# akavkl/Automated-Recycling-Sorter-with-Vision-Transformers

Measured on NVIDIA B200. Metric: vit_b16_224_inference_images_per_sec, higher is better.
Workload: dtype bf16

## Files before the change

automated-recycling-sorter-with-vision-transformers_b200/csrc/common.cu:

```cuda
#include "common.h"

#include <cstdarg>
#include <cstring>
#include <atomic>
#include <mutex>
#include <vector>

namespace vitk {

static thread_local char g_err[1024] = "";
static std::atomic<long long> g_launches{0};

int set_error(int code, const char* fmt, ...) {
  va_list ap;
  va_start(ap, fmt);
  vsnprintf(g_err, sizeof(g_err), fmt, ap);
  va_end(ap);
  return code;
}
const char* last_error() { return g_err; }

void count_launch() { g_launches.fetch_add(1, std::memory_order_relaxed); }
long long launch_count() { return g_launches.load(std::memory_order_relaxed); }

// ... 86 lines not shown
  cudaGetDevice(&dev);
  if (!g_dev_init[dev]) init_dev(dev);
  const int n = g_sm_count[dev] - g_sm_reserve;
  return n < 2 ? 2 : n;
}
int device_cc() {
  int dev = 0;
  cudaGetDevice(&dev);
  if (!g_dev_init[dev]) init_dev(dev);
  return g_cc[dev];
}

typedef CUresult (*EncodeTiledFn)(CUtensorMap*, CUtensorMapDataType, cuuint32_t, void*,
                                  const cuuint64_t*, const cuuint64_t*, const cuuint32_t*,
                                  const cuuint32_t*, CUtensorMapInterleave, CUtensorMapSwizzle,
                                  CUtensorMapL2promotion, CUtensorMapFloatOOBfill);
static EncodeTiledFn g_encode = nullptr;
static std::once_flag g_encode_once;

static EncodeTiledFn get_encode() {
  std::call_once(g_encode_once, [] {
    void* fn = nullptr;
    cudaDriverEntryPointQueryResult qres;
    if (cudaGetDriverEntryPoint("cuTensorMapEncodeTiled", &fn, cudaEnableDefault, &qres) ==
            cudaSuccess &&
        qres == cudaDriverEntryPointSuccess)
      g_encode = reinterpret_cast<EncodeTiledFn>(fn);
  });
  return g_encode;
}

int make_tmap_2d(CUtensorMap* out, const void* base, int elem_bytes, uint64_t inner,
                 uint64_t outer, uint64_t pitch_bytes, uint32_t box_inner, uint32_t box_outer,
                 bool swizzle128) {
  EncodeTiledFn enc = get_encode();
  if (!enc) return set_error(VITK_ERR_CUDA, "cuTensorMapEncodeTiled entry point not available");
  if ((reinterpret_cast<uintptr_t>(base) & 15) != 0 || (pitch_bytes & 15) != 0)
    return set_error(VITK_ERR_INVALID,
                     "TMA operand must be 16-byte aligned (base %p, pitch %llu bytes)", base,
                     (unsigned long long)pitch_bytes);
  if (box_inner * (uint32_t)elem_bytes > 128 && swizzle128)
    return set_error(VITK_ERR_INVALID, "128B-swizzled TMA box inner extent exceeds 128 bytes");
  if (box_outer > 256 || box_inner > 256)
    return set_error(VITK_ERR_INVALID, "TMA box extent exceeds 256");
  CUtensorMapDataType dt;
  switch (elem_bytes) {
    case 2: dt = CU_TENSOR_MAP_DATA_TYPE_BFLOAT16; break;
    case 4: dt = CU_TENSOR_MAP_DATA_TYPE_FLOAT32; break;
    default: return set_error(VITK_ERR_INVALID, "unsupported TMA element size %d", elem_bytes);
  }
  cuuint64_t dims[2] = {inner, outer};
  cuuint64_t strides[1] = {pitch_bytes};
  cuuint32_t box[2] = {box_inner, box_outer};
  cuuint32_t estr[2] = {1, 1};
  CUresult r = enc(out, dt, 2, const_cast<void*>(base), dims, strides, box, estr,
                   CU_TENSOR_MAP_INTERLEAVE_NONE,
                   swizzle128 ? CU_TENSOR_MAP_SWIZZLE_128B : CU_TENSOR_MAP_SWIZZLE_NONE,
                   CU_TENSOR_MAP_L2_PROMOTION_L2_256B, CU_TENSOR_MAP_FLOAT_OOB_FILL_NONE);
  if (r != CUDA_SUCCESS)
    return set_error(VITK_ERR_CUDA,
                     "cuTensorMapEncodeTiled failed (%d): base %p dims {%llu,%llu} pitch %llu box "
                     "{%u,%u}",
                     (int)r, base, (unsigned long long)inner, (unsigned long long)outer,
                     (unsigned long long)pitch_bytes, box_inner, box_outer);
  return VITK_OK;
}

int make_tmap_3d(CUtensorMap* out, const void* base, int elem_bytes, uint64_t inner, uint64_t rows,
                 uint64_t batch, uint64_t row_pitch_bytes, uint64_t batch_pitch_bytes,
                 uint32_t box_inner, uint32_t box_rows) {
  EncodeTiledFn enc = get_encode();
  if (!enc) return set_error(VITK_ERR_CUDA, "cuTensorMapEncodeTiled entry point not available");
  if ((reinterpret_cast<uintptr_t>(base) & 15) != 0 || (row_pitch_bytes & 15) != 0 ||
      (batch_pitch_bytes & 15) != 0)
    return set_error(VITK_ERR_INVALID, "TMA operand must be 16-byte aligned");
  if (box_inner * (uint32_t)elem_bytes != 128 || box_rows > 256 || box_rows == 0)
    return set_error(VITK_ERR_INVALID, "bad 3-D TMA box {%u,%u}", box_inner, box_rows);
  CUtensorMapDataType dt;
  switch (elem_bytes) {
    case 2: dt = CU_TENSOR_MAP_DATA_TYPE_BFLOAT16; break;
    case 4: dt = CU_TENSOR_MAP_DATA_TYPE_FLOAT32; break;
    default: return set_error(VITK_ERR_INVALID, "unsupported TMA element size %d", elem_bytes);
  }
  cuuint64_t dims[3] = {inner, rows, batch};
  cuuint64_t strides[2] = {row_pitch_bytes, batch_pitch_bytes};
  cuuint32_t box[3] = {box_inner, box_rows, 1};
  cuuint32_t estr[3] = {1, 1, 1};
  CUresult r = enc(out, dt, 3, const_cast<void*>(base), dims, strides, box, estr,
                   CU_TENSOR_MAP_INTERLEAVE_NONE, CU_TENSOR_MAP_SWIZZLE_128B,
                   CU_TENSOR_MAP_L2_PROMOTION_L2_256B, CU_TENSOR_MAP_FLOAT_OOB_FILL_NONE);
  if (r != CUDA_SUCCESS)
// ... 6 lines not shown
```

automated-recycling-sorter-with-vision-transformers_b200/csrc/common.h:

```cpp
#pragma once
#include <cstddef>
#include <cstdint>
#include <cstdio>
#include <cuda.h>
#include <cuda_runtime.h>

#include "../../include/vitk.h"

namespace vitk {


int set_error(int code, const char* fmt, ...);
const char* last_error();

#define VITK_CHECK_CUDA(expr)                                                              \
  do {                                                                                     \
    cudaError_t _e = (expr);                                                               \
    if (_e != cudaSuccess)                                                                 \
      return ::vitk::set_error(VITK_ERR_CUDA, "%s failed: %s (%s:%d)", #expr,      \
                               cudaGetErrorString(_e), __FILE__, __LINE__);                \
  } while (0)

#define VITK_CHECK_LAUNCH(name)                                                            \
  do {                                                                                     \
// ... 26 lines not shown
  explicit Carver(void* b) : base(static_cast<char*>(b)) {}
  void* take(size_t n) {
    void* p = base ? base + off : nullptr;
    off += align_up(n, 1024);
    return p;
  }
};

enum ProfKind : int { PROF_GEMM = 0, PROF_ATTN = 1, PROF_LN = 2, PROF_PATCH = 3, PROF_OTHER = 4,
                      PROF_OPT = 5, PROF_NKINDS = 6 };
bool profile_enabled();
void profile_enable(bool on);
int profile_collect(double* ms, double* work, long long* launches, int nkinds);

struct ProfileScope {
  ProfileScope(int kind, double work, cudaStream_t stream);
  ~ProfileScope();
  int idx_;
  cudaStream_t stream_;
};

struct SweepAlternation {
  SweepAlternation();
  ~SweepAlternation();
};
int sweep_next();

int sm_count();
void reserve_sms(int n);
int device_cc();

int make_tmap_2d(CUtensorMap* out, const void* base, int elem_bytes, uint64_t inner,
                 uint64_t outer, uint64_t pitch_bytes, uint32_t box_inner, uint32_t box_outer,
                 bool swizzle128 = true);

int make_tmap_3d(CUtensorMap* out, const void* base, int elem_bytes, uint64_t inner, uint64_t rows,
                 uint64_t batch, uint64_t row_pitch_bytes, uint64_t batch_pitch_bytes,
                 uint32_t box_inner, uint32_t box_rows);

}
```

automated-recycling-sorter-with-vision-transformers_b200/csrc/gemm_sm100.cu:

```cuda
#include "gemm_sm100.cuh"

#include <mutex>

#include "common.h"
#include "ptx.cuh"
#include "rowops.cuh"
#include "train_ops.cuh"

namespace vitk {
using namespace ptx;

#ifdef VITK_GEMM_TRACE
__device__ long long g_gemm_trace[160][8];
#define GT_BEGIN(v) const long long v = clock64()
#define GT_ADD(acc, v) acc += clock64() - v
#else
#define GT_BEGIN(v) do { } while (0)
#define GT_ADD(acc, v) do { } while (0)
#endif

namespace {

constexpr int kBlockM = 128;
constexpr int kBlockK = 64;
constexpr int kUmmaK = 16;
constexpr int kNumEpiWarps = 8;
constexpr int kFirstEpiWarp = 4;
constexpr int kNumThreads = (kFirstEpiWarp + kNumEpiWarps) * 32;
constexpr int kAccStages = 2;

template <int BLOCK_N, int CTAS, int SLABS = 2>
struct Cfg {
  static constexpr int kStagingPerWarp = SLABS * 4096;
  static constexpr int kStagingBytes = kNumEpiWarps * kStagingPerWarp;
  static constexpr int kABytes = kBlockM * kBlockK * 2;
  static constexpr int kBRows = BLOCK_N / CTAS;
  static constexpr int kBBytes = kBRows * kBlockK * 2;
  static constexpr int kStageBytes = kABytes + kBBytes;
  static constexpr int kBarBytes = 1024;
  static constexpr int kBudget = 232448 - 1024 - kBarBytes - kStagingBytes;
  static constexpr int kStages = kBudget / kStageBytes > 8 ? 8 : kBudget / kStageBytes;
  static constexpr int kTmemCols = kAccStages * BLOCK_N;
  static constexpr int kSmemBytes =
      kStages * kStageBytes + kStagingBytes + kBarBytes + 1024;
  static_assert(kStages >= 3, "pipeline too shallow");
  static_assert(kSmemBytes <= 232448, "exceeds 227 KB of shared memory");
  static constexpr int kNumBars = 2 * kStages + 2 * kAccStages + 1 + 2 * kNumEpiWarps;
  static_assert(8 * kNumBars <= kBarBytes, "barrier block too small");
};

__device__ __forceinline__ float gelu_erf(float x) {
  return 0.5f * x * (1.f + erff(x * 0.70710678118654752440f));
}
__device__ __forceinline__ float gelu_fast(float x) {
  const float x2 = fminf(x * x, 100.f);
  const float p = fmaf(x2, fmaf(x2, 9.2473074e-4f, -0.10595751f), -2.3019681f);
  float e, r;
  asm("ex2.approx.ftz.f32 %0, %1;" : "=f"(e) : "f"(x * p));
  asm("rcp.approx.ftz.f32 %0, %1;" : "=f"(r) : "f"(1.f + e));
  return x * r;
}
__device__ __forceinline__ float gelu_fast_tanh(float x) {
  const float x2 = fminf(x * x, 64.f);
  const float p = fmaf(x2, fmaf(x2, -3.5651449e-4f, 0.037011533f), 0.79753114f);
  float t;
  asm("tanh.approx.f32 %0, %1;" : "=f"(t) : "f"(x * p));
  return x * fmaf(0.5f, t, 0.5f);
}
__device__ __forceinline__ float gelu_grad_fast(float x) {
  const float x2 = fminf(x * x, 100.f);
  const float p = fmaf(x2, fmaf(x2, 9.2473074e-4f, -0.10595751f), -2.3019681f);
  float e, phi;
  asm("ex2.approx.ftz.f32 %0, %1;" : "=f"(e) : "f"(x * p));
  asm("rcp.approx.ftz.f32 %0, %1;" : "=f"(phi) : "f"(1.f + e));
  const float gp = fmaf(x2, fmaf(x2, -3.20487363e-3f, 0.22033243f), 1.5956033f);
  return fmaf(x * phi, (1.f - phi) * gp, phi);
}
__device__ __forceinline__ void gelu_fast_tanh_pair(float& a, float& b) {
// ... 188 lines not shown
        o.x = x[4 * j + 0] + r.x;
        o.y = x[4 * j + 1] + r.y;
        o.z = x[4 * j + 2] + r.z;
        o.w = x[4 * j + 3] + r.w;
        reinterpret_cast<float4*>(out)[j] = o;
      }
    } else {
      _Pragma("unroll") for (int j = 0; j < 32; ++j)
        if (n0 + j < N) out[j] = x[j] + res[j];
    }
  } else if constexpr (EPI == EPI_F32) {
    float* out = reinterpret_cast<float*>(e.out) + static_cast<size_t>(m) * e.ldo + n0;
    const float beta = e.beta;
    if (full) {
#pragma unroll
      for (int j = 0; j < 8; ++j) {
        float4 o = make_float4(x[4 * j + 0], x[4 * j + 1], x[4 * j + 2], x[4 * j + 3]);
        if (beta != 0.f) {
          const float4 p = reinterpret_cast<const float4*>(out)[j];
          o.x = fmaf(beta, p.x, o.x);
          o.y = fmaf(beta, p.y, o.y);
          o.z = fmaf(beta, p.z, o.z);
          o.w = fmaf(beta, p.w, o.w);
        }
        reinterpret_cast<float4*>(out)[j] = o;
      }
    } else {
      _Pragma("unroll") for (int j = 0; j < 32; ++j)
        if (n0 + j < N) out[j] = (beta != 0.f) ? fmaf(beta, out[j], x[j]) : x[j];
    }
  }
}

template <int EPI>
__device__ __forceinline__ void acc_plus_bias(const uint32_t (&v)[32], int n0, int N,
                                              const GemmEpilogue& e, float (&x)[32]) {
  float acc_scale = 1.f;
  if constexpr (EPI == EPI_F32) acc_scale = e.alpha;
  if (n0 + 32 <= N) {
    if (e.bias != nullptr) {
      const float4* b4 = reinterpret_cast<const float4*>(e.bias + n0);
#pragma unroll
      for (int j = 0; j < 8; ++j) {
        const float4 b = __ldg(b4 + j);
#ifdef VITK_SCALAR_BIAS
        if constexpr (true) {
#else
        if constexpr (EPI == EPI_F32) {
#endif
          x[4 * j + 0] = fmaf(acc_scale, __uint_as_float(v[4 * j + 0]), b.x);
          x[4 * j + 1] = fmaf(acc_scale, __uint_as_float(v[4 * j + 1]), b.y);
          x[4 * j + 2] = fmaf(acc_scale, __uint_as_float(v[4 * j + 2]), b.z);
          x[4 * j + 3] = fmaf(acc_scale, __uint_as_float(v[4 * j + 3]), b.w);
        } else {
          unpack2(fadd2(pack2(v[4 * j + 0], v[4 * j + 1]), pack2f(b.x, b.y)), x[4 * j + 0],
                  x[4 * j + 1]);
          unpack2(fadd2(pack2(v[4 * j + 2], v[4 * j + 3]), pack2f(b.z, b.w)), x[4 * j + 2],
                  x[4 * j + 3]);
        }
      }
    } else {
#pragma unroll
      for (int j = 0; j < 32; ++j) x[j] = acc_scale * __uint_as_float(v[j]);
    }
  } else {
#pragma unroll
    for (int j = 0; j < 32; ++j) {
      const float b = (e.bias != nullptr && n0 + j < N) ? __ldg(e.bias + n0 + j) : 0.f;
      x[j] = fmaf(acc_scale, __uint_as_float(v[j]), b);
    }
  }
}

__device__ __forceinline__ void acc_scale_bias(const uint32_t (&v)[32], int n0, int N,
                                               const GemmEpilogue& e, float rstd, float (&x)[32]) {
  if (n0 + 32 <= N) {
    const float4* b4 = reinterpret_cast<const float4*>(e.bias + n0);
    const uint64_t r2 = pack2f(rstd, rstd);
#pragma unroll
    for (int j = 0; j < 8; ++j) {
      const float4 b = __ldg(b4 + j);
      unpack2(ffma2(r2, pack2(v[4 * j + 0], v[4 * j + 1]), pack2f(b.x, b.y)), x[4 * j + 0],
              x[4 * j + 1]);
      unpack2(ffma2(r2, pack2(v[4 * j + 2], v[4 * j + 3]), pack2f(b.z, b.w)), x[4 * j + 2],
              x[4 * j + 3]);
    }
  } else {
#pragma unroll
    for (int j = 0; j < 32; ++j) {
      const float b = (n0 + j < N) ? __ldg(e.bias + n0 + j) : 0.f;
      x[j] = fmaf(rstd, __uint_as_float(v[j]), b);
    }
  }
}

__device__ __forceinline__ void resid_chunk_staged(const uint32_t (&v)[32], int row0, int n0, int M,
                                                   int N, const GemmEpilogue& e, uint32_t slab,
                                                   int lane) {
  float x[32];
  acc_plus_bias<EPI_RESID_F32>(v, n0, N, e, x);
  if (e.drop.thresh != 0u)
    drop_apply_run<32>(x, static_cast<uint32_t>(row0 + lane) * static_cast<uint32_t>(N) +
                              static_cast<uint32_t>(n0), e.drop);
  const uint32_t row = slab + static_cast<uint32_t>(lane) * 128u;
#pragma unroll
  for (int j = 0; j < 8; ++j)
    st_shared_v4(row + (static_cast<uint32_t>(j ^ (lane & 7)) << 4), __float_as_uint(x[4 * j]),
                 __float_as_uint(x[4 * j + 1]), __float_as_uint(x[4 * j + 2]),
                 __float_as_uint(x[4 * j + 3]));
  __syncwarp();
  const int piece = lane & 7;
  const bool col_ok = n0 + 4 * piece < N;
  const bool vec_ok = aligned16(e.out) && aligned16(e.resid);
#pragma unroll
  for (int it = 0; it < 8; ++it) {
    const int r = it * 4 + (lane >> 3);
    const int m = row0 + r;
    if (m < M && col_ok) {
      int out_row = m, res_row = m;
      if (e.rows_per_group > 0) {
        const int g = m / e.rows_per_group;
        const int rr = m - g * e.rows_per_group;
// ... 16 lines not shown
        o[0] = a0 + rs[0];
        o[1] = a1 + rs[1];
        o[2] = a2 + rs[2];
        o[3] = a3 + rs[3];
      }
    }
  }
  __syncwarp();
}

__device__ __forceinline__ void stage_and_store(const uint32_t (&pk)[32], uint32_t stg, int& buf,
                                                int lane, const CUtensorMap* tmap, int c0, int c1,
                                                bool reduce) {
  if (lane == 0) tma_store_wait_read<1>();
  __syncwarp();
  const uint32_t slab = stg + static_cast<uint32_t>(buf) * 4096u;
  const uint32_t row = slab + static_cast<uint32_t>(lane) * 128u;
#pragma unroll
  for (int j = 0; j < 8; ++j)
    st_shared_v4(row + (static_cast<uint32_t>(j ^ (lane & 7)) << 4), pk[4 * j], pk[4 * j + 1],
                 pk[4 * j + 2], pk[4 * j + 3]);
  fence_proxy_async_smem();
  __syncwarp();
  if (lane == 0) {
    if (reduce)
      tma_reduce_add_2d(tmap, slab, c0, c1);
    else
      tma_store_2d(tmap, slab, c0, c1);
    tma_store_commit();
  }
  buf ^= 1;
}

template <int BLOCK_N, int EPI, int CTAS, bool TMA_EPI, bool MN>
__global__ void __launch_bounds__(kNumThreads, 1)
gemm_tn_kernel(const __grid_constant__ CUtensorMap tmap_a,
               const __grid_constant__ CUtensorMap tmap_b,
               const __grid_constant__ CUtensorMap tmap_c,
               const __grid_constant__ CUtensorMap tmap_c2, int M, int N, int K,
               int kb_per_split, int num_splits, int descending,
               const __grid_constant__ GemmEpilogue e) {
  constexpr bool kAuxTma = TMA_EPI && (EPI == EPI_DGELU_BF16);
  constexpr bool kStats = TMA_EPI && (EPI == EPI_RESID_STATS_F32);
  static_assert(EPI != EPI_RESID_STATS_F32 || TMA_EPI, "the statistics epilogue is TMA-only");
  using C = Cfg<BLOCK_N, CTAS, kAuxTma ? 3 : 2>;
  constexpr int kStagingBytes = C::kStagingBytes;
  constexpr int kStagingPerWarp = C::kStagingPerWarp;
  constexpr int kTileM = kBlockM * CTAS;
  extern __shared__ uint8_t smem_raw[];
  const uint32_t raw_addr = smem_u32(smem_raw);
  const uint32_t base = (raw_addr + 1023u) & ~1023u;
  uint8_t* smem = smem_raw + (base - raw_addr);

  const uint32_t staging_base = base + C::kStages * C::kStageBytes;
  const uint32_t bar_base = staging_base + kStagingBytes;
  auto full_bar = [&](int s) { return bar_base + 8u * s; };
  auto empty_bar = [&](int s) { return bar_base + 8u * (C::kStages + s); };
  auto tfull_bar = [&](int a) { return bar_base + 8u * (2 * C::kStages + a); };
  auto tempty_bar = [&](int a) { return bar_base + 8u * (2 * C::kStages + kAccStages + a); };
  volatile uint32_t* tmem_slot = reinterpret_cast<volatile uint32_t*>(
      smem + C::kStages * C::kStageBytes + kStagingBytes + 8 * (2 * C::kStages + 2 * kAccStages));
  auto aux_bar = [&](int w) { return bar_base + 8u * (2 * C::kStages + 2 * kAccStages + 1 + w); };
  [[maybe_unused]] auto aux2_bar = [&](int w) {
    return bar_base + 8u * (2 * C::kStages + 2 * kAccStages + 1 + kNumEpiWarps + w);
  };

  const int warp = threadIdx.x >> 5;
  const int lane = threadIdx.x & 31;
  const uint32_t cta_rank = (CTAS == 2) ? cluster_ctarank() : 0u;
  const bool is_leader = (cta_rank == 0);
  const int cluster_id = blockIdx.x / CTAS;
  const int num_clusters = gridDim.x / CTAS;

  const int num_m_tiles = (M + kTileM - 1) / kTileM;
  const int num_n_tiles = (N + BLOCK_N - 1) / BLOCK_N;
  const int num_out_tiles = num_m_tiles * num_n_tiles;
  const int num_tiles = num_out_tiles * num_splits;
  const int num_kb_total = (K + kBlockK - 1) / kBlockK;
// ... 78 lines not shown
                tma_load_2d(sa + j * 8192, &tmap_a, fbar, m0 + 64 * j, kb * kBlockK);
            }
#pragma unroll
            for (int j = 0; j < C::kBRows / 64; ++j) {
              if constexpr (CTAS == 2)
                tma_load_2d_2sm(sb + j * 8192, &tmap_b, fbar, n0 + 64 * j, kb * kBlockK);
              else
                tma_load_2d(sb + j * 8192, &tmap_b, fbar, n0 + 64 * j, kb * kBlockK);
            }
          }
          if (++stage == C::kStages) {
            stage = 0;
            phase ^= 1u;
          }
        }
      }
      if constexpr (CTAS == 2) {
        for (int s = 0; s < C::kStages; ++s) {
          mbar_wait(empty_bar(stage), phase ^ 1u);
          if (++stage == C::kStages) {
            stage = 0;
            phase ^= 1u;
          }
        }
      }
    }
  } else if (warp == 1) {
    if (is_leader) {
      constexpr uint32_t idesc = make_idesc_bf16(kTileM, BLOCK_N, MN ? 1 : 0, MN ? 1 : 0);
      int stage = 0;
      uint32_t phase = 0;
      int acc = 0;
      uint32_t acc_phase = 0;
      [[maybe_unused]] long long gt_full = 0, gt_empty = 0;
      GT_BEGIN(gt_start);
      for (int work = cluster_id; work < num_tiles; work += num_clusters) {
        GT_BEGIN(gt_e);
        mbar_wait(tempty_bar(acc), acc_phase ^ 1u);
        GT_ADD(gt_empty, gt_e);
        tc_fence_after();
        const uint32_t d_tmem = tmem_base + static_cast<uint32_t>(acc * BLOCK_N);
        const int kb0 = kb_begin(work);
        for (int kb = kb0; kb < kb_end(work); ++kb) {
          GT_BEGIN(gt_f);
          mbar_wait(full_bar(stage), phase);
          GT_ADD(gt_full, gt_f);
          tc_fence_after();
          const uint32_t sa = base + stage * C::kStageBytes;
          const uint32_t sb = sa + C::kABytes;
          const uint64_t a_desc = make_desc_sw128(sa, MN ? 8192 : 16, 1024);
          const uint64_t b_desc = make_desc_sw128(sb, MN ? 8192 : 16, 1024);
          constexpr uint32_t kstep = MN ? 128u : 2u;
          if (elect_one_sync()) {
#pragma unroll
            for (int k = 0; k < kBlockK / kUmmaK; ++k) {
              const uint32_t accum = (kb > kb0 || k > 0) ? 1u : 0u;
              if constexpr (CTAS == 2)
                mma_bf16_ss_2sm(d_tmem, a_desc + kstep * k, b_desc + kstep * k, idesc, accum);
              else
                mma_bf16_ss(d_tmem, a_desc + kstep * k, b_desc + kstep * k, idesc, accum);
            }
            if constexpr (CTAS == 2) mma_commit_2sm_mc(empty_bar(stage), 3);
            else mma_commit(empty_bar(stage));
          }
          __syncwarp();
          if (++stage == C::kStages) {
            stage = 0;
            phase ^= 1u;
          }
        }
        if (elect_one_sync()) {
          if constexpr (CTAS == 2) mma_commit_2sm_mc(tfull_bar(acc), 3);
          else mma_commit(tfull_bar(acc));
        }
        __syncwarp();
        if (++acc == kAccStages) {
          acc = 0;
          acc_phase ^= 1u;
        }
      }
#ifdef VITK_GEMM_TRACE
      if (lane == 0 && cluster_id < 160) {
        g_gemm_trace[cluster_id][0] = clock64() - gt_start;
        g_gemm_trace[cluster_id][1] = gt_full;
        g_gemm_trace[cluster_id][2] = gt_empty;
        g_gemm_trace[cluster_id][3] = (num_tiles - cluster_id + num_clusters - 1) / num_clusters;
      }
#endif
    }
  } else if (warp >= kFirstEpiWarp) {
    const int q = warp & 3;
    const int half = (warp - kFirstEpiWarp) >> 2;
    constexpr int kColsPerWarp = BLOCK_N / 2;
    const int slab_row = static_cast<int>(cta_rank) * kBlockM + q * 32;
    const uint32_t stg = staging_base + static_cast<uint32_t>(warp - kFirstEpiWarp) * kStagingPerWarp;
    int buf = 0;
    int acc = 0;
    uint32_t acc_phase = 0;
    [[maybe_unused]] uint32_t aux_phase = 0;
    [[maybe_unused]] const uint32_t aux_slab = stg + 2u * 4096u;
    [[maybe_unused]] const uint32_t my_aux_bar = aux_bar(warp - kFirstEpiWarp);
    [[maybe_unused]] const uint32_t my_aux2_bar = aux2_bar(warp - kFirstEpiWarp);
    [[maybe_unused]] uint32_t x_phase = 0;
    [[maybe_unused]] long long gt_epi_wait = 0, gt_epi_ld = 0, gt_epi_math = 0, gt_epi_store = 0;
    [[maybe_unused]] float2 ln_next[8];
    [[maybe_unused]] float ln_rstd_next = 1.f;
    [[maybe_unused]] bool ln_have_next = false;
    [[maybe_unused]] auto ln_load_stats = [&](int m, float2 (&t)[8]) {
#pragma unroll
      for (int p2 = 0; p2 < 8; ++p2) {
        t[p2] = make_float2(0.f, 0.f);
        if (p2 < e.ln_nparts && m < M)
          asm volatile("ld.global.nc.v2.f32 {%0, %1}, [%2];"
                       : "=f"(t[p2].x), "=f"(t[p2].y)
                       : "l"(e.ln_part + static_cast<size_t>(p2) * M + m));
      }
    };
    [[maybe_unused]] auto ln_finish = [&](float s1, float s2) {
      const float inv_d = 1.f / static_cast<float>(e.ln_dim);
      const float mean = s1 * inv_d;
      const float var = fmaxf(fmaf(-mean, mean, s2 * inv_d), 0.f);
      return rsqrtf(var + e.ln_eps);
    };
    for (int work = cluster_id; work < num_tiles; work += num_clusters) {
      const int tile = tile_of(work);
      const int m_blk = tile / num_n_tiles;
      const int n_blk = tile - m_blk * num_n_tiles;
      if constexpr (kAuxTma) {
        const int r0 = m_blk * kTileM + slab_row;
        const int c0 = n_blk * BLOCK_N + half * kColsPerWarp;
        if (lane == 0 && r0 < M && c0 < N) {
          mbar_arrive_expect_tx(my_aux_bar, 4096);
          tma_load_2d(aux_slab, &tmap_c2, my_aux_bar, c0, r0);
        }
      }
      const int row0 = m_blk * kTileM + slab_row;
      if constexpr (kStats) {
        if (lane == 0 && row0 < M) {
          tma_store_wait_read<0>();
#pragma unroll
          for (int c = 0; c < 2; ++c) {
            const int c0 = n_blk * BLOCK_N + half * kColsPerWarp + 32 * c;
            if (c0 < N) {
              const uint32_t xb = c == 0 ? my_aux_bar : my_aux2_bar;
              mbar_arrive_expect_tx(xb, 4096);
              tma_load_2d(stg + static_cast<uint32_t>(c) * 4096u, &tmap_c, xb, c0, row0);
            }
          }
        }
      }
      [[maybe_unused]] float ln_rstd = 1.f;
      if constexpr (TMA_EPI && (EPI == EPI_BF16 || is_gelu_epi<EPI>())) {
        if (e.ln_part != nullptr) {
          if (ln_have_next) {
            ln_rstd = ln_rstd_next;
          } else {
            float s1 = 0.f, s2 = 0.f;
            ln_load_stats(row0 + lane, ln_next);
#pragma unroll
            for (int p2 = 0; p2 < 8; ++p2) {
              s1 += ln_next[p2].x;
              s2 += ln_next[p2].y;
            }
            ln_rstd = ln_finish(s1, s2);
          }
          const int work_nx = work + num_clusters;
          ln_have_next = work_nx < num_tiles;
          if (ln_have_next)
            ln_load_stats((tile_of(work_nx) / num_n_tiles) * kTileM + slab_row + lane, ln_next);
        }
      }
      GT_BEGIN(gt_w);
      mbar_wait(tfull_bar(acc), acc_phase);
      GT_ADD(gt_epi_wait, gt_w);
      tc_fence_after();
      const uint32_t t_row = tmem_base + (static_cast<uint32_t>(q * 32) << 16) +
                             static_cast<uint32_t>(acc * BLOCK_N + half * kColsPerWarp);
      const int n_base = n_blk * BLOCK_N + half * kColsPerWarp;
      auto release_acc = [&]() {
        tc_fence_before();
        __syncwarp();
        if (lane == 0) {
          if (CTAS == 2 && !is_leader)
            mbar_arrive_cluster(mapa_shared(tempty_bar(acc), 0));
          else
            mbar_arrive(tempty_bar(acc));
        }
      };
      if constexpr (kStats) {
        const bool o2_wide =
            ((reinterpret_cast<uintptr_t>(e.out2) | static_cast<uintptr_t>(e.ldo * 2)) & 31u) == 0;
        float sum1 = 0.f, sum2 = 0.f;
        uint32_t v[2][32];
        tmem_ld_32x32b_x32(t_row, v[0]);
#pragma unroll
        for (int c = 0; c < kColsPerWarp / 32; ++c) {
          tmem_ld_wait();
          if (c + 1 < kColsPerWarp / 32) tmem_ld_32x32b_x32(t_row + (c + 1) * 32, v[(c + 1) & 1]);
          else release_acc();
          const int n0 = n_base + c * 32;
          if (row0 < M && n0 < N) {
            float x[32];
            acc_plus_bias<EPI>(v[c & 1], n0, N, e, x);
            const uint32_t slab = stg + static_cast<uint32_t>(c & 1) * 4096u;
            const uint32_t row = slab + static_cast<uint32_t>(lane) * 128u;
            mbar_wait((c & 1) ? my_aux2_bar : my_aux_bar, (x_phase >> (c & 1)) & 1u);
            x_phase ^= 1u << (c & 1);
#pragma unroll
            for (int j = 0; j < 8; ++j) {
              float r0, r1, r2, r3;
              asm volatile("ld.shared.v4.f32 {%0,%1,%2,%3}, [%4];"
// ... 55 lines not shown
              const uint32_t xb = (c & 1) ? my_aux2_bar : my_aux_bar;
              mbar_arrive_expect_tx(xb, 4096);
              tma_load_2d(slab, &tmap_c, xb, n0 + 64, row0);
            }
          }
        }
        if (row0 + lane < M && n_base < N)
          e.ln_part_out[static_cast<size_t>(n_base / kColsPerWarp) * M + (row0 + lane)] =
              make_float2(sum1, sum2);
      } else if constexpr (TMA_EPI) {
        constexpr bool kOutF32 = (EPI == EPI_RESID_F32 || EPI == EPI_F32);
        if constexpr (kOutF32) {
          const bool reduce = (EPI == EPI_RESID_F32) || (e.beta != 0.f);
          uint32_t v[2][32];
          tmem_ld_32x32b_x32(t_row, v[0]);
#pragma unroll
          for (int c = 0; c < kColsPerWarp / 32; ++c) {
            tmem_ld_wait();
            if (c + 1 < kColsPerWarp / 32) tmem_ld_32x32b_x32(t_row + (c + 1) * 32, v[(c + 1) & 1]);
            else release_acc();
            const int n0 = n_base + c * 32;
            if (row0 < M && n0 < N) {
              float x[32];
              acc_plus_bias<EPI>(v[c & 1], n0, N, e, x);
              if constexpr (EPI == EPI_RESID_F32) {
                if (e.drop.thresh != 0u)
                  drop_apply_run<32>(x, static_cast<uint32_t>(row0 + lane) * static_cast<uint32_t>(N) +
                                            static_cast<uint32_t>(n0), e.drop);
              }
              uint32_t pk[32];
#pragma unroll
              for (int j = 0; j < 32; ++j) pk[j] = __float_as_uint(x[j]);
              stage_and_store(pk, stg, buf, lane, &tmap_c, n0, row0, reduce);
            }
          }
        } else {
#pragma unroll 1
          for (int g = 0; g < kColsPerWarp / 64; ++g) {
            uint32_t v0[32], v1[32];
            GT_BEGIN(gt_l);
            tmem_ld_32x32b_x32(t_row + g * 64, v0);
            tmem_ld_32x32b_x32(t_row + g * 64 + 32, v1);
            tmem_ld_wait();
            if (g + 1 == kColsPerWarp / 64) release_acc();
            GT_ADD(gt_epi_ld, gt_l);
            GT_BEGIN(gt_m);
            const int n0 = n_base + g * 64;
            if (row0 < M && n0 < N) {
              float x0[32], x1[32];
              if (e.ln_part != nullptr) {
                acc_scale_bias(v0, n0, N, e, ln_rstd, x0);
                acc_scale_bias(v1, n0 + 32, N, e, ln_rstd, x1);
              } else {
                acc_plus_bias<EPI>(v0, n0, N, e, x0);
                acc_plus_bias<EPI>(v1, n0 + 32, N, e, x1);
              }
              uint32_t pk[32];
              [[maybe_unused]] const uint32_t drop_idx0 =
                  static_cast<uint32_t>(row0 + lane) * static_cast<uint32_t>(N) +
                  static_cast<uint32_t>(n0);
              if constexpr (EPI == EPI_DGELU_BF16) {
                if (e.drop.thresh != 0u) {
                  drop_apply_run<32>(x0, drop_idx0, e.drop);
                  drop_apply_run<32>(x1, drop_idx0 + 32u, e.drop);
                }
              }
              if constexpr (kAuxTma) {
                mbar_wait(my_aux_bar, aux_phase);
                aux_phase ^= 1u;
                uint32_t a[32];
                const uint32_t arow = aux_slab + static_cast<uint32_t>(lane) * 128u;
#pragma unroll
                for (int j = 0; j < 8; ++j)
                  asm volatile("ld.shared.v4.b32 {%0,%1,%2,%3}, [%4];"
                               : "=r"(a[4 * j]), "=r"(a[4 * j + 1]), "=r"(a[4 * j + 2]),
                                 "=r"(a[4 * j + 3])
                               : "r"(arow + (static_cast<uint32_t>(j ^ (lane & 7)) << 4))
                               : "memory");
                __syncwarp();
                const int n_next = n0 + 64;
                if (lane == 0 && g + 1 < kColsPerWarp / 64 && n_next < N) {
                  mbar_arrive_expect_tx(my_aux_bar, 4096);
                  tma_load_2d(aux_slab, &tmap_c2, my_aux_bar, n_next, row0);
                }
#pragma unroll
                for (int j = 0; j < 16; ++j) {
                  dgelu_tanh_pair(x0[2 * j], x0[2 * j + 1], bf16lo_to_f32(a[j]), bf16hi_to_f32(a[j]));
                  dgelu_tanh_pair(x1[2 * j], x1[2 * j + 1], bf16lo_to_f32(a[16 + j]),
                                  bf16hi_to_f32(a[16 + j]));
                }
              }
              if constexpr (is_gelu_epi<EPI>()) {
                if (e.out2 != nullptr) {
#pragma unroll
                  for (int j = 0; j < 16; ++j) {
                    pk[j] = pack_bf16x2(x0[2 * j], x0[2 * j + 1]);
                    pk[16 + j] = pack_bf16x2(x1[2 * j], x1[2 * j + 1]);
                  }
                  stage_and_store(pk, stg, buf, lane, &tmap_c2, n0, row0, false);
                }
                if constexpr (EPI == EPI_RELU_BF16) {
#pragma unroll
                  for (int j = 0; j < 32; ++j) {
                    x0[j] = fmaxf(x0[j], 0.f);
                    x1[j] = fmaxf(x1[j], 0.f);
                  }
                } else if constexpr (EPI == EPI_GELU_TANH_BF16) {
#pragma unroll
                  for (int j = 0; j < 16; ++j) {
                    gelu_fast_tanh_pair(x0[2 * j], x0[2 * j + 1]);
                    gelu_fast_tanh_pair(x1[2 * j], x1[2 * j + 1]);
                  }
                } else {
#pragma unroll
                  for (int j = 0; j < 16; ++j) {
                    gelu_fast_pair(x0[2 * j], x0[2 * j + 1]);
                    gelu_fast_pair(x1[2 * j], x1[2 * j + 1]);
                  }
                }
                if (e.drop.thresh != 0u) {
                  drop_apply_run<32>(x0, drop_idx0, e.drop);
                  drop_apply_run<32>(x1, drop_idx0 + 32u, e.drop);
                }
              }
#pragma unroll
              for (int j = 0; j < 16; ++j) {
                pk[j] = pack_bf16x2(x0[2 * j], x0[2 * j + 1]);
                pk[16 + j] = pack_bf16x2(x1[2 * j], x1[2 * j + 1]);
              }
              GT_ADD(gt_epi_math, gt_m);
              GT_BEGIN(gt_s);
              stage_and_store(pk, stg, buf, lane, &tmap_c, n0, row0, false);
              GT_ADD(gt_epi_store, gt_s);
            }
          }
        }
      } else {
        const int m = row0 + lane;
        uint32_t v[2][32];
        tmem_ld_32x32b_x32(t_row, v[0]);
#pragma unroll
        for (int c = 0; c < kColsPerWarp / 32; ++c) {
          tmem_ld_wait();
          if (c + 1 < kColsPerWarp / 32) tmem_ld_32x32b_x32(t_row + (c + 1) * 32, v[(c + 1) & 1]);
          else release_acc();
          const int n0 = n_base + c * 32;
          if constexpr (EPI == EPI_RESID_F32) {
            if (row0 < M && n0 < N) resid_chunk_staged(v[c & 1], row0, n0, M, N, e, stg, lane);
          } else {
            if (m < M && n0 < N) epilogue_chunk<EPI>(v[c & 1], m, n0, N, e);
          }
// ... 12 lines not shown
            s2 += ln_next[p2].y;
          }
          ln_rstd_next = ln_finish(s1, s2);
        }
      }
    }
#ifdef VITK_GEMM_TRACE
    if (lane == 0 && warp == kFirstEpiWarp && is_leader && cluster_id < 160) {
      g_gemm_trace[cluster_id][4] = gt_epi_wait;
      g_gemm_trace[cluster_id][5] = gt_epi_ld;
      g_gemm_trace[cluster_id][6] = gt_epi_math;
      g_gemm_trace[cluster_id][7] = gt_epi_store;
    }
#endif
    if constexpr (TMA_EPI) {
      if (lane == 0) tma_store_wait<0>();
    }
  }

  tc_fence_before();
  if constexpr (CTAS == 2) cluster_sync_all(); else __syncthreads();
  if (warp == 2) {
    tc_fence_after();
    if constexpr (CTAS == 2) tmem_dealloc_2sm(tmem_base, C::kTmemCols);
    else tmem_dealloc(tmem_base, C::kTmemCols);
  }
}

int g_force_ctas = 0;
int g_force_direct_epi = 0;

template <int BLOCK_N, int EPI, int CTAS, bool TMA_EPI, bool MN>
int launch(const GemmProblem& p, cudaStream_t stream) {
  using C = Cfg<BLOCK_N, CTAS, (TMA_EPI && EPI == EPI_DGELU_BF16) ? 3 : 2>;
  auto kernel = gemm_tn_kernel<BLOCK_N, EPI, CTAS, TMA_EPI, MN>;
  static std::once_flag once;
  static cudaError_t attr_err = cudaSuccess;
  std::call_once(once, [&] {
    attr_err = cudaFuncSetAttribute(kernel, cudaFuncAttributeMaxDynamicSharedMemorySize,
                                    C::kSmemBytes);
  });
  if (attr_err != cudaSuccess)
    return set_error(VITK_ERR_CUDA, "cudaFuncSetAttribute(gemm smem %d) failed: %s", C::kSmemBytes,
                     cudaGetErrorString(attr_err));
  CUtensorMap ta, tb, tc, tc2;
  if constexpr (MN) {
    VITK_TRY(make_tmap_2d(&ta, p.A, 2, (uint64_t)p.M, (uint64_t)p.K, (uint64_t)p.lda * 2, 64, 64));
    VITK_TRY(make_tmap_2d(&tb, p.B, 2, (uint64_t)p.N, (uint64_t)p.K, (uint64_t)p.ldb * 2, 64, 64));
  } else {
    VITK_TRY(make_tmap_2d(&ta, p.A, 2, (uint64_t)p.K, (uint64_t)p.M, (uint64_t)p.lda * 2, kBlockK,
                          kBlockM));
    VITK_TRY(make_tmap_2d(&tb, p.B, 2, (uint64_t)p.K, (uint64_t)p.N, (uint64_t)p.ldb * 2, kBlockK,
                          C::kBRows));
  }
  if constexpr (TMA_EPI) {
    constexpr bool kOutF32 =
        (EPI == EPI_RESID_F32 || EPI == EPI_F32 || EPI == EPI_RESID_STATS_F32);
    constexpr int eb = kOutF32 ? 4 : 2;
    VITK_TRY(make_tmap_2d(&tc, p.e.out, eb, (uint64_t)p.N, (uint64_t)p.M, (uint64_t)p.e.ldo * eb,
                          128 / eb, 32));
    tc2 = tc;
    if (is_gelu_epi<EPI>() && p.e.out2 != nullptr)
      VITK_TRY(make_tmap_2d(&tc2, p.e.out2, eb, (uint64_t)p.N, (uint64_t)p.M,
                            (uint64_t)p.e.ldo * eb, 128 / eb, 32));
    if (EPI == EPI_DGELU_BF16)
      VITK_TRY(make_tmap_2d(&tc2, p.e.aux, 2, (uint64_t)p.N, (uint64_t)p.M, (uint64_t)p.e.ldo * 2,
                            64, 32));
  } else {
    tc = ta;
    tc2 = ta;
  }
  const int tile_m = kBlockM * CTAS;
  const int num_kb = (p.K + kBlockK - 1) / kBlockK;
  int splits = p.split_k < 1 ? 1 : p.split_k;
  if (splits > num_kb) splits = num_kb;
  const int kb_per_split = (num_kb + splits - 1) / splits;
  splits = (num_kb + kb_per_split - 1) / kb_per_split;
  const int num_tiles = ((p.M + tile_m - 1) / tile_m) * ((p.N + BLOCK_N - 1) / BLOCK_N) * splits;
  int grid = sm_count();
  if (grid <= 0) return set_error(VITK_ERR_NO_DEVICE, "no CUDA device");
  grid = grid / CTAS * CTAS;
  if (num_tiles * CTAS < grid) grid = num_tiles * CTAS;
  cudaLaunchConfig_t cfg = {};
  cfg.gridDim = dim3(grid);
  cfg.blockDim = dim3(kNumThreads);
  cfg.dynamicSmemBytes = C::kSmemBytes;
  cfg.stream = stream;
  cudaLaunchAttribute attr;
  attr.id = cudaLaunchAttributeClusterDimension;
  attr.val.clusterDim.x = CTAS;
  attr.val.clusterDim.y = 1;
  attr.val.clusterDim.z = 1;
  cfg.attrs = &attr;
  cfg.numAttrs = 1;
  ProfileScope prof(PROF_GEMM, 2.0 * p.M * p.N * p.K, stream);
  const int descending = sweep_next();
  cudaError_t le = cudaLaunchKernelEx(&cfg, kernel, ta, tb, tc, tc2, p.M, p.N, p.K, kb_per_split,
                                      splits, descending, p.e);
  if (le != cudaSuccess)
    return set_error(VITK_ERR_CUDA, "launch of gemm_tn_kernel<%d,%d,%d,%d,%d> failed: %s", BLOCK_N,
                     EPI, CTAS, (int)TMA_EPI, (int)MN, cudaGetErrorString(le));
  VITK_CHECK_LAUNCH("gemm_tn_kernel");
  return VITK_OK;
}

template <int EPI, bool TMA_EPI, bool MN>
int dispatch_tile(const GemmProblem& p, cudaStream_t stream) {
  const int waste256 = ((p.N + 255) / 256) * 256 - p.N;
  const int waste128 = ((p.N + 127) / 128) * 128 - p.N;
  const bool n128 = waste128 < waste256;
  int ctas = (p.M > kBlockM) ? 2 : 1;
  if (g_force_ctas == 1 || g_force_ctas == 2) ctas = g_force_ctas;
  if (ctas == 2)
    return n128 ? launch<128, EPI, 2, TMA_EPI, MN>(p, stream)
                : launch<256, EPI, 2, TMA_EPI, MN>(p, stream);
  constexpr bool kTma1 = TMA_EPI && (EPI != EPI_DGELU_BF16);
  return n128 ? launch<128, EPI, 1, kTma1, MN>(p, stream)
              : launch<256, EPI, 1, kTma1, MN>(p, stream);
// ... 283 lines not shown
```

Baseline: 25210.

## Use sixteen epilogue warps with 64-byte swizzled staging for GELU GEMMs

For TMA-epilogue GELU GEMMs, the kernel now runs 16 epilogue warps instead of 8. Each warp drains a narrower column slice of the TMEM accumulator in 16-column chunks and stages results into smaller 2 KB slabs with 64-byte swizzle, or 128-byte swizzle when a warp owns a full 64-column slice. The aim is to spread the heavy GELU math and stores across more warps so the epilogue keeps pace with the tensor-core mainloop. To support this, make_tmap_2d gains a selectable swizzle width, and the per-config thread count now flows through Cfg and the launch bounds. The trade-offs are more registers and threads per CTA, plus extra TMA store instructions.

```diff
diff --git a/automated-recycling-sorter-with-vision-transformers_b200/csrc/common.cu b/automated-recycling-sorter-with-vision-transformers_b200/csrc/common.cu
--- a/automated-recycling-sorter-with-vision-transformers_b200/csrc/common.cu
+++ b/automated-recycling-sorter-with-vision-transformers_b200/csrc/common.cu
@@ -142,15 +142,23 @@
 
 int make_tmap_2d(CUtensorMap* out, const void* base, int elem_bytes, uint64_t inner,
                  uint64_t outer, uint64_t pitch_bytes, uint32_t box_inner, uint32_t box_outer,
-                 bool swizzle128) {
+                 int swizzle_bytes) {
   EncodeTiledFn enc = get_encode();
   if (!enc) return set_error(VITK_ERR_CUDA, "cuTensorMapEncodeTiled entry point not available");
   if ((reinterpret_cast<uintptr_t>(base) & 15) != 0 || (pitch_bytes & 15) != 0)
     return set_error(VITK_ERR_INVALID,
                      "TMA operand must be 16-byte aligned (base %p, pitch %llu bytes)", base,
                      (unsigned long long)pitch_bytes);
-  if (box_inner * (uint32_t)elem_bytes > 128 && swizzle128)
-    return set_error(VITK_ERR_INVALID, "128B-swizzled TMA box inner extent exceeds 128 bytes");
+  CUtensorMapSwizzle swizzle;
+  switch (swizzle_bytes) {
+    case 0: swizzle = CU_TENSOR_MAP_SWIZZLE_NONE; break;
+    case 64: swizzle = CU_TENSOR_MAP_SWIZZLE_64B; break;
+    case 128: swizzle = CU_TENSOR_MAP_SWIZZLE_128B; break;
+    default: return set_error(VITK_ERR_INVALID, "unsupported TMA swizzle width %d", swizzle_bytes);
+  }
+  if (swizzle_bytes != 0 && box_inner * (uint32_t)elem_bytes > (uint32_t)swizzle_bytes)
+    return set_error(VITK_ERR_INVALID, "TMA box inner extent exceeds its %d-byte swizzle",
+                     swizzle_bytes);
   if (box_outer > 256 || box_inner > 256)
     return set_error(VITK_ERR_INVALID, "TMA box extent exceeds 256");
   CUtensorMapDataType dt;
@@ -165,8 +173,7 @@
   cuuint32_t estr[2] = {1, 1};
   CUresult r = enc(out, dt, 2, const_cast<void*>(base), dims, strides, box, estr,
                    CU_TENSOR_MAP_INTERLEAVE_NONE,
-                   swizzle128 ? CU_TENSOR_MAP_SWIZZLE_128B : CU_TENSOR_MAP_SWIZZLE_NONE,
-                   CU_TENSOR_MAP_L2_PROMOTION_L2_256B, CU_TENSOR_MAP_FLOAT_OOB_FILL_NONE);
+                   swizzle, CU_TENSOR_MAP_L2_PROMOTION_L2_256B, CU_TENSOR_MAP_FLOAT_OOB_FILL_NONE);
   if (r != CUDA_SUCCESS)
     return set_error(VITK_ERR_CUDA,
                      "cuTensorMapEncodeTiled failed (%d): base %p dims {%llu,%llu} pitch %llu box "
diff --git a/automated-recycling-sorter-with-vision-transformers_b200/csrc/common.h b/automated-recycling-sorter-with-vision-transformers_b200/csrc/common.h
--- a/automated-recycling-sorter-with-vision-transformers_b200/csrc/common.h
+++ b/automated-recycling-sorter-with-vision-transformers_b200/csrc/common.h
@@ -82,7 +82,7 @@
 
 int make_tmap_2d(CUtensorMap* out, const void* base, int elem_bytes, uint64_t inner,
                  uint64_t outer, uint64_t pitch_bytes, uint32_t box_inner, uint32_t box_outer,
-                 bool swizzle128 = true);
+                 int swizzle_bytes = 128);
 
 int make_tmap_3d(CUtensorMap* out, const void* base, int elem_bytes, uint64_t inner, uint64_t rows,
                  uint64_t batch, uint64_t row_pitch_bytes, uint64_t batch_pitch_bytes,
diff --git a/automated-recycling-sorter-with-vision-transformers_b200/csrc/gemm_sm100.cu b/automated-recycling-sorter-with-vision-transformers_b200/csrc/gemm_sm100.cu
--- a/automated-recycling-sorter-with-vision-transformers_b200/csrc/gemm_sm100.cu
+++ b/automated-recycling-sorter-with-vision-transformers_b200/csrc/gemm_sm100.cu
@@ -12,8 +12,8 @@
 
 #ifdef VITK_GEMM_TRACE
 __device__ long long g_gemm_trace[160][8];
-#define GT_BEGIN(v) const long long v = clock64()
-#define GT_ADD(acc, v) acc += clock64() - v
+#define GT_BEGIN(v) const uint32_t v = static_cast<uint32_t>(clock())
+#define GT_ADD(acc, v) acc += static_cast<uint32_t>(clock()) - v
 #else
 #define GT_BEGIN(v) do { } while (0)
 #define GT_ADD(acc, v) do { } while (0)
@@ -24,14 +24,24 @@
 constexpr int kBlockM = 128;
 constexpr int kBlockK = 64;
 constexpr int kUmmaK = 16;
-constexpr int kNumEpiWarps = 8;
 constexpr int kFirstEpiWarp = 4;
-constexpr int kNumThreads = (kFirstEpiWarp + kNumEpiWarps) * 32;
 constexpr int kAccStages = 2;
 
-template <int BLOCK_N, int CTAS, int SLABS = 2>
+constexpr int epi_warps(int epi, bool tma_epi) {
+#ifdef VITK_EPI16_BF16
+  return tma_epi && (epi == EPI_BF16 || epi == EPI_GELU_BF16 || epi == EPI_GELU_TANH_BF16) ? 16 : 8;
+#else
+  return tma_epi && (epi == EPI_GELU_BF16 || epi == EPI_GELU_TANH_BF16) ? 16 : 8;
+#endif
+}
+
+template <int BLOCK_N, int EPI, int CTAS, bool TMA_EPI>
 struct Cfg {
-  static constexpr int kStagingPerWarp = SLABS * 4096;
+  static constexpr int kNumEpiWarps = epi_warps(EPI, TMA_EPI);
+  static constexpr int kNumThreads = (kFirstEpiWarp + kNumEpiWarps) * 32;
+  static constexpr int kSlabBytes = kNumEpiWarps == 16 ? 2048 : 4096;
+  static constexpr int kSlabs = (TMA_EPI && EPI == EPI_DGELU_BF16) ? 3 : 2;
+  static constexpr int kStagingPerWarp = kSlabs * kSlabBytes;
   static constexpr int kStagingBytes = kNumEpiWarps * kStagingPerWarp;
   static constexpr int kABytes = kBlockM * kBlockK * 2;
   static constexpr int kBRows = BLOCK_N / CTAS;
@@ -44,6 +54,8 @@
   static constexpr int kSmemBytes =
       kStages * kStageBytes + kStagingBytes + kBarBytes + 1024;
   static_assert(kStages >= 3, "pipeline too shallow");
+  static_assert(BLOCK_N != 256 || CTAS != 2 || kSlabs != 2 || kStages == 5,
+                "the 256 x 256 pair tiles keep a 5-stage operand ring");
   static_assert(kSmemBytes <= 232448, "exceeds 227 KB of shared memory");
   static constexpr int kNumBars = 2 * kStages + 2 * kAccStages + 1 + 2 * kNumEpiWarps;
   static_assert(8 * kNumBars <= kBarBytes, "barrier block too small");
@@ -298,16 +310,16 @@
   }
 }
 
-template <int EPI>
-__device__ __forceinline__ void acc_plus_bias(const uint32_t (&v)[32], int n0, int N,
-                                              const GemmEpilogue& e, float (&x)[32]) {
+template <int EPI, int W>
+__device__ __forceinline__ void acc_plus_bias(const uint32_t (&v)[W], int n0, int N,
+                                              const GemmEpilogue& e, float (&x)[W]) {
   float acc_scale = 1.f;
   if constexpr (EPI == EPI_F32) acc_scale = e.alpha;
-  if (n0 + 32 <= N) {
+  if (n0 + W <= N) {
     if (e.bias != nullptr) {
       const float4* b4 = reinterpret_cast<const float4*>(e.bias + n0);
 #pragma unroll
-      for (int j = 0; j < 8; ++j) {
+      for (int j = 0; j < W / 4; ++j) {
         const float4 b = __ldg(b4 + j);
 #ifdef VITK_SCALAR_BIAS
         if constexpr (true) {
@@ -327,24 +339,25 @@
       }
     } else {
 #pragma unroll
-      for (int j = 0; j < 32; ++j) x[j] = acc_scale * __uint_as_float(v[j]);
+      for (int j = 0; j < W; ++j) x[j] = acc_scale * __uint_as_float(v[j]);
     }
   } else {
 #pragma unroll
-    for (int j = 0; j < 32; ++j) {
+    for (int j = 0; j < W; ++j) {
       const float b = (e.bias != nullptr && n0 + j < N) ? __ldg(e.bias + n0 + j) : 0.f;
       x[j] = fmaf(acc_scale, __uint_as_float(v[j]), b);
     }
   }
 }
 
-__device__ __forceinline__ void acc_scale_bias(const uint32_t (&v)[32], int n0, int N,
-                                               const GemmEpilogue& e, float rstd, float (&x)[32]) {
-  if (n0 + 32 <= N) {
+template <int W>
+__device__ __forceinline__ void acc_scale_bias(const uint32_t (&v)[W], int n0, int N,
+                                               const GemmEpilogue& e, float rstd, float (&x)[W]) {
+  if (n0 + W <= N) {
     const float4* b4 = reinterpret_cast<const float4*>(e.bias + n0);
     const uint64_t r2 = pack2f(rstd, rstd);
 #pragma unroll
-    for (int j = 0; j < 8; ++j) {
+    for (int j = 0; j < W / 4; ++j) {
       const float4 b = __ldg(b4 + j);
       unpack2(ffma2(r2, pack2(v[4 * j + 0], v[4 * j + 1]), pack2f(b.x, b.y)), x[4 * j + 0],
               x[4 * j + 1]);
@@ -353,7 +366,7 @@
     }
   } else {
 #pragma unroll
-    for (int j = 0; j < 32; ++j) {
+    for (int j = 0; j < W; ++j) {
       const float b = (n0 + j < N) ? __ldg(e.bias + n0 + j) : 0.f;
       x[j] = fmaf(rstd, __uint_as_float(v[j]), b);
     }
@@ -436,8 +449,21 @@
   buf ^= 1;
 }
 
+template <int ROW_BYTES>
+__device__ __forceinline__ void stage_16_cols(const uint32_t (&pk)[8], uint32_t slab, int u0,
+                                              int lane) {
+  static_assert(ROW_BYTES == 64 || ROW_BYTES == 128, "64- or 128-byte swizzle");
+  const uint32_t row = slab + static_cast<uint32_t>(lane) * ROW_BYTES;
+  const uint32_t swz = ROW_BYTES == 128 ? static_cast<uint32_t>(lane & 7)
+                                         : static_cast<uint32_t>(lane >> 1) & 3u;
+#pragma unroll
+  for (int j = 0; j < 2; ++j)
+    st_shared_v4(row + (((static_cast<uint32_t>(u0) + j) ^ swz) << 4), pk[4 * j], pk[4 * j + 1],
+                 pk[4 * j + 2], pk[4 * j + 3]);
+}
+
 template <int BLOCK_N, int EPI, int CTAS, bool TMA_EPI, bool MN>
-__global__ void __launch_bounds__(kNumThreads, 1)
+__global__ void __launch_bounds__((kFirstEpiWarp + epi_warps(EPI, TMA_EPI)) * 32, 1)
 gemm_tn_kernel(const __grid_constant__ CUtensorMap tmap_a,
                const __grid_constant__ CUtensorMap tmap_b,
                const __grid_constant__ CUtensorMap tmap_c,
@@ -447,7 +473,8 @@
   constexpr bool kAuxTma = TMA_EPI && (EPI == EPI_DGELU_BF16);
   constexpr bool kStats = TMA_EPI && (EPI == EPI_RESID_STATS_F32);
   static_assert(EPI != EPI_RESID_STATS_F32 || TMA_EPI, "the statistics epilogue is TMA-only");
-  using C = Cfg<BLOCK_N, CTAS, kAuxTma ? 3 : 2>;
+  using C = Cfg<BLOCK_N, EPI, CTAS, TMA_EPI>;
+  constexpr int kNumEpiWarps = C::kNumEpiWarps;
   constexpr int kStagingBytes = C::kStagingBytes;
   constexpr int kStagingPerWarp = C::kStagingPerWarp;
   constexpr int kTileM = kBlockM * CTAS;
@@ -592,7 +619,7 @@
       uint32_t phase = 0;
       int acc = 0;
       uint32_t acc_phase = 0;
-      [[maybe_unused]] long long gt_full = 0, gt_empty = 0;
+      [[maybe_unused]] uint32_t gt_full = 0, gt_empty = 0;
       GT_BEGIN(gt_start);
       for (int work = cluster_id; work < num_tiles; work += num_clusters) {
         GT_BEGIN(gt_e);
@@ -641,7 +668,7 @@
       }
 #ifdef VITK_GEMM_TRACE
       if (lane == 0 && cluster_id < 160) {
-        g_gemm_trace[cluster_id][0] = clock64() - gt_start;
+        g_gemm_trace[cluster_id][0] = static_cast<uint32_t>(clock()) - gt_start;
         g_gemm_trace[cluster_id][1] = gt_full;
         g_gemm_trace[cluster_id][2] = gt_empty;
         g_gemm_trace[cluster_id][3] = (num_tiles - cluster_id + num_clusters - 1) / num_clusters;
@@ -650,19 +677,19 @@
     }
   } else if (warp >= kFirstEpiWarp) {
     const int q = warp & 3;
-    const int half = (warp - kFirstEpiWarp) >> 2;
-    constexpr int kColsPerWarp = BLOCK_N / 2;
+    const int slice = (warp - kFirstEpiWarp) >> 2;
+    constexpr int kColsPerWarp = BLOCK_N / (kNumEpiWarps / 4);
     const int slab_row = static_cast<int>(cta_rank) * kBlockM + q * 32;
     const uint32_t stg = staging_base + static_cast<uint32_t>(warp - kFirstEpiWarp) * kStagingPerWarp;
     int buf = 0;
     int acc = 0;
     uint32_t acc_phase = 0;
     [[maybe_unused]] uint32_t aux_phase = 0;
-    [[maybe_unused]] const uint32_t aux_slab = stg + 2u * 4096u;
+    [[maybe_unused]] const uint32_t aux_slab = stg + 2u * C::kSlabBytes;
     [[maybe_unused]] const uint32_t my_aux_bar = aux_bar(warp - kFirstEpiWarp);
     [[maybe_unused]] const uint32_t my_aux2_bar = aux2_bar(warp - kFirstEpiWarp);
     [[maybe_unused]] uint32_t x_phase = 0;
-    [[maybe_unused]] long long gt_epi_wait = 0, gt_epi_ld = 0, gt_epi_math = 0, gt_epi_store = 0;
+    [[maybe_unused]] uint32_t gt_epi_wait = 0, gt_epi_ld = 0, gt_epi_math = 0, gt_epi_store = 0;
     [[maybe_unused]] float2 ln_next[8];
     [[maybe_unused]] float ln_rstd_next = 1.f;
     [[maybe_unused]] bool ln_have_next = false;
@@ -688,7 +715,7 @@
       const int n_blk = tile - m_blk * num_n_tiles;
       if constexpr (kAuxTma) {
         const int r0 = m_blk * kTileM + slab_row;
-        const int c0 = n_blk * BLOCK_N + half * kColsPerWarp;
+        const int c0 = n_blk * BLOCK_N + slice * kColsPerWarp;
         if (lane == 0 && r0 < M && c0 < N) {
           mbar_arrive_expect_tx(my_aux_bar, 4096);
           tma_load_2d(aux_slab, &tmap_c2, my_aux_bar, c0, r0);
@@ -700,7 +727,7 @@
           tma_store_wait_read<0>();
 #pragma unroll
           for (int c = 0; c < 2; ++c) {
-            const int c0 = n_blk * BLOCK_N + half * kColsPerWarp + 32 * c;
+            const int c0 = n_blk * BLOCK_N + slice * kColsPerWarp + 32 * c;
             if (c0 < N) {
               const uint32_t xb = c == 0 ? my_aux_bar : my_aux2_bar;
               mbar_arrive_expect_tx(xb, 4096);
@@ -735,8 +762,8 @@
       GT_ADD(gt_epi_wait, gt_w);
       tc_fence_after();
       const uint32_t t_row = tmem_base + (static_cast<uint32_t>(q * 32) << 16) +
-                             static_cast<uint32_t>(acc * BLOCK_N + half * kColsPerWarp);
-      const int n_base = n_blk * BLOCK_N + half * kColsPerWarp;
+                             static_cast<uint32_t>(acc * BLOCK_N + slice * kColsPerWarp);
+      const int n_base = n_blk * BLOCK_N + slice * kColsPerWarp;
       auto release_acc = [&]() {
         tc_fence_before();
         __syncwarp();
@@ -858,6 +885,76 @@
 #pragma unroll
               for (int j = 0; j < 32; ++j) pk[j] = __float_as_uint(x[j]);
               stage_and_store(pk, stg, buf, lane, &tmap_c, n0, row0, reduce);
+            }
+          }
+        } else if constexpr (kNumEpiWarps == 16) {
+          constexpr int kSub = kColsPerWarp / 16;
+          static_assert(kSub % 2 == 0, "a warp's slice is whole 32-column slabs");
+          const bool with_out2 = is_gelu_epi<EPI>() && e.out2 != nullptr;
+          const bool wide = kColsPerWarp == 64 && !with_out2;
+          uint32_t v[2][16];
+          tmem_ld_32x32b_x16(t_row, v[0]);
+#pragma unroll
+          for (int c = 0; c < kSub; ++c) {
+            GT_BEGIN(gt_l);
+            tmem_ld_wait();
+            if (c + 1 < kSub) tmem_ld_32x32b_x16(t_row + (c + 1) * 16, v[(c + 1) & 1]);
+            else release_acc();
+            GT_ADD(gt_epi_ld, gt_l);
+            const int nc = wide ? n_base : n_base + (c >> 1) * 32;
+            const bool first = wide ? c == 0 : (c & 1) == 0;
+            const bool last = wide ? c == kSub - 1 : (c & 1) == 1;
+            if (row0 < M && nc < N) {
+              GT_BEGIN(gt_m);
+              const int n0 = n_base + c * 16;
+              const uint32_t slab_o2 = stg;
+              const uint32_t slab =
+                  stg + (wide ? 0u : (with_out2 ? 1u : static_cast<uint32_t>(buf)) * 2048u);
+              float x[16];
+              if (e.ln_part != nullptr) acc_scale_bias(v[c & 1], n0, N, e, ln_rstd, x);
+              else acc_plus_bias<EPI>(v[c & 1], n0, N, e, x);
+              if (first) {
+                if (lane == 0) {
+                  if (wide || with_out2) tma_store_wait_read<0>();
+                  else tma_store_wait_read<1>();
+                }
+                __syncwarp();
+              }
+              uint32_t pk[8];
+              if constexpr (is_gelu_epi<EPI>()) {
+                if (with_out2) {
+#pragma unroll
+                  for (int j = 0; j < 8; ++j) pk[j] = pack_bf16x2(x[2 * j], x[2 * j + 1]);
+                  stage_16_cols<64>(pk, slab_o2, 2 * (c & 1), lane);
+                }
+                if constexpr (EPI == EPI_GELU_TANH_BF16) {
+#pragma unroll
+                  for (int j = 0; j < 8; ++j) gelu_fast_tanh_pair(x[2 * j], x[2 * j + 1]);
+                } else {
+#pragma unroll
+                  for (int j = 0; j < 8; ++j) gelu_fast_pair(x[2 * j], x[2 * j + 1]);
+                }
+                if (e.drop.thresh != 0u)
+                  drop_apply_run<16>(x, static_cast<uint32_t>(row0 + lane) * static_cast<uint32_t>(N) +
+                                            static_cast<uint32_t>(n0), e.drop);
+              }
+#pragma unroll
+              for (int j = 0; j < 8; ++j) pk[j] = pack_bf16x2(x[2 * j], x[2 * j + 1]);
+              GT_ADD(gt_epi_math, gt_m);
+              GT_BEGIN(gt_s);
+              if (wide) stage_16_cols<128>(pk, slab, 2 * c, lane);
+              else stage_16_cols<64>(pk, slab, 2 * (c & 1), lane);
+              if (last) {
+                fence_proxy_async_smem();
+                __syncwarp();
+                if (lane == 0) {
+                  if (with_out2) tma_store_2d(&tmap_c2, slab_o2, nc, row0);
+                  tma_store_2d(&tmap_c, slab, nc, row0);
+                  tma_store_commit();
+                }
+                buf ^= 1;
+              }
+              GT_ADD(gt_epi_store, gt_s);
             }
           }
         } else {
@@ -916,7 +1013,7 @@
                                   bf16hi_to_f32(a[16 + j]));
                 }
               }
-              if constexpr (is_gelu_epi<EPI>()) {
+              if constexpr (EPI == EPI_RELU_BF16) {
                 if (e.out2 != nullptr) {
 #pragma unroll
                   for (int j = 0; j < 16; ++j) {
@@ -925,24 +1022,10 @@
                   }
                   stage_and_store(pk, stg, buf, lane, &tmap_c2, n0, row0, false);
                 }
-                if constexpr (EPI == EPI_RELU_BF16) {
-#pragma unroll
-                  for (int j = 0; j < 32; ++j) {
-                    x0[j] = fmaxf(x0[j], 0.f);
-                    x1[j] = fmaxf(x1[j], 0.f);
-                  }
-                } else if constexpr (EPI == EPI_GELU_TANH_BF16) {
-#pragma unroll
-                  for (int j = 0; j < 16; ++j) {
-                    gelu_fast_tanh_pair(x0[2 * j], x0[2 * j + 1]);
-                    gelu_fast_tanh_pair(x1[2 * j], x1[2 * j + 1]);
-                  }
-                } else {
-#pragma unroll
-                  for (int j = 0; j < 16; ++j) {
-                    gelu_fast_pair(x0[2 * j], x0[2 * j + 1]);
-                    gelu_fast_pair(x1[2 * j], x1[2 * j + 1]);
-                  }
+#pragma unroll
+                for (int j = 0; j < 32; ++j) {
+                  x0[j] = fmaxf(x0[j], 0.f);
+                  x1[j] = fmaxf(x1[j], 0.f);
                 }
                 if (e.drop.thresh != 0u) {
                   drop_apply_run<32>(x0, drop_idx0, e.drop);
@@ -1021,7 +1104,7 @@
 
 template <int BLOCK_N, int EPI, int CTAS, bool TMA_EPI, bool MN>
 int launch(const GemmProblem& p, cudaStream_t stream) {
-  using C = Cfg<BLOCK_N, CTAS, (TMA_EPI && EPI == EPI_DGELU_BF16) ? 3 : 2>;
+  using C = Cfg<BLOCK_N, EPI, CTAS, TMA_EPI>;
   auto kernel = gemm_tn_kernel<BLOCK_N, EPI, CTAS, TMA_EPI, MN>;
   static std::once_flag once;
   static cudaError_t attr_err = cudaSuccess;
@@ -1046,12 +1129,14 @@
     constexpr bool kOutF32 =
         (EPI == EPI_RESID_F32 || EPI == EPI_F32 || EPI == EPI_RESID_STATS_F32);
     constexpr int eb = kOutF32 ? 4 : 2;
+    const bool with_out2 = is_gelu_epi<EPI>() && p.e.out2 != nullptr;
+    const int row_bytes = (C::kNumEpiWarps == 8 || (BLOCK_N == 256 && !with_out2)) ? 128 : 64;
     VITK_TRY(make_tmap_2d(&tc, p.e.out, eb, (uint64_t)p.N, (uint64_t)p.M, (uint64_t)p.e.ldo * eb,
-                          128 / eb, 32));
+                          row_bytes / eb, 32, row_bytes));
     tc2 = tc;
-    if (is_gelu_epi<EPI>() && p.e.out2 != nullptr)
+    if (with_out2)
       VITK_TRY(make_tmap_2d(&tc2, p.e.out2, eb, (uint64_t)p.N, (uint64_t)p.M,
-                            (uint64_t)p.e.ldo * eb, 128 / eb, 32));
+                            (uint64_t)p.e.ldo * eb, row_bytes / eb, 32, row_bytes));
     if (EPI == EPI_DGELU_BF16)
       VITK_TRY(make_tmap_2d(&tc2, p.e.aux, 2, (uint64_t)p.N, (uint64_t)p.M, (uint64_t)p.e.ldo * 2,
                             64, 32));
@@ -1072,7 +1157,7 @@
   if (num_tiles * CTAS < grid) grid = num_tiles * CTAS;
   cudaLaunchConfig_t cfg = {};
   cfg.gridDim = dim3(grid);
-  cfg.blockDim = dim3(kNumThreads);
+  cfg.blockDim = dim3(C::kNumThreads);
   cfg.dynamicSmemBytes = C::kSmemBytes;
   cfg.stream = stream;
   cudaLaunchAttribute attr;
```

Result: faster. 25860, median of 6 (+2.6%).
